# zbqq/neus2

Hardware: AMD Instinct MI355X
Metric: training samples/sec (compacted NeuS2 training samples, DTU-scan24-shaped synthetic, base.json) (higher is better)
Workload: dtype fp16 MFMA (fp32 accumulate) / fp32 optimizer; 1 GPU; NeuS2 train step, Config S, base.json L=14 T=2^19 W=64, Nc=2^18/GPU, R=2^18/GPU fixed, all 14 levels active (network trained 800 steps before the warm-up); global_batch=262144, rays_per_gpu=262144, parallelism=dp1, prepare_steps=800, levels_active=14

## Files before the change

### include/neus2_hip.h

```cpp
#ifndef NEUS2_HIP_H
#define NEUS2_HIP_H

#include <stdint.h>

#ifdef __cplusplus
extern "C" {
#endif

typedef struct NeusTestbed NeusTestbed;

typedef struct NeusNetworkConfig {
	uint32_t n_levels;
	uint32_t n_features_per_level;
	uint32_t log2_hashmap_size;
	uint32_t base_resolution;
	float per_level_scale;
	float top_resolution;
	float valid_level_scale;
	float base_valid_level_scale;
	uint32_t base_training_step;
	uint32_t n_neurons;
	uint32_t n_density_hidden;
	uint32_t n_rgb_hidden;
	float learning_rate, beta1, beta2, epsilon, l2_reg;
// ... 147 lines not shown
	float learning_rate_factor;
} NeusOptimizerState;
int neus_testbed_get_optimizer_state(NeusTestbed* tb, NeusOptimizerState* st, float* m1, float* m2, uint32_t* steps, uint16_t* ema_half);
int neus_testbed_set_optimizer_state(NeusTestbed* tb, const NeusOptimizerState* st, const float* m1, const float* m2, const uint32_t* steps,
                                     const uint16_t* ema_half);
int neus_testbed_set_training_options(NeusTestbed* tb, const NeusTrainingOptions* opts);
int neus_testbed_set_progressive_inference(NeusTestbed* tb, int mode, const uint32_t* chunk_ends, uint32_t n_ends);
int neus_testbed_ray_counts(NeusTestbed* tb, uint32_t n, uint32_t* nreq, uint32_t* ccount, uint32_t* numsteps );
int neus_debug_time_kernel(NeusTestbed* tb, int kernel, int variant, int iters, float* ms_out);
int neus_testbed_time_kernel(NeusTestbed* tb, int kernel, int iters, float* ms_out, uint32_t* units_out);
int neus_debug_march_stats(NeusTestbed* tb, uint32_t n, uint32_t* out);
int neus_debug_march_profile(NeusTestbed* tb, unsigned long long* out, uint32_t max_waves, uint32_t* n_waves);
int neus_debug_scatter_stats(NeusTestbed* tb, uint64_t* records_per_level, uint32_t* max_region);
int neus_debug_scatter_parts(NeusTestbed* tb, uint32_t* parts_per_level );
int neus_debug_grid_scatter(NeusTestbed* tb, void* hip_stream, uint32_t n_cap, const uint32_t* n_valid, const float* coords,
                            uint32_t coord_stride, uint32_t valid_level, const void* dLdenc, const void* genc, const float* v,
                            float* grid_grad_out);
int neus_debug_exclusive_scan(void* hip_stream, const uint32_t* in, uint32_t* out, uint32_t n, int reps, uint32_t* failures);
int neus_debug_scan_giveup(void* hip_stream, const uint32_t* in, uint32_t* out, uint32_t n, uint32_t* failures);
int neus_debug_inject_health(NeusTestbed* tb, uint32_t flags);
int neus_debug_set_lds_fill(NeusTestbed* tb, uint32_t pattern);
int neus_debug_set_lds_fill_all(NeusTestbed* tb, uint32_t pattern);
int neus_debug_set_xcd_shift(NeusTestbed* tb, uint32_t n_blocks);
int neus_debug_get_batch(NeusTestbed* tb, float* coords_out, uint16_t* dl_dout_out, float* loss_out);
int neus_debug_denorm_probe(int device, uint32_t n, uint32_t launches, uint64_t* stats);
int neus_debug_get_buffer(NeusTestbed* tb, int id, uint64_t offset, uint64_t nbytes, void* host);
int neus_debug_replay_loss_grad(NeusTestbed* tb, uint16_t* dl_dout_out);
int neus_debug_sample_rays_round0(NeusTestbed* tb, void* stream, uint32_t n_rays, uint32_t n_rays_total, uint64_t rng_state, uint64_t rng_inc,
                                  uint32_t max_samples, const uint8_t* bitfield, float* rays, uint32_t* numsteps, float* coords,
                                  uint32_t* counters_out, uint32_t chunk_end, uint32_t* list, uint32_t* list_len, uint32_t lds_fill);
int neus_testbed_stream(NeusTestbed* tb, void** hip_stream);
int neus_testbed_synchronize(NeusTestbed* tb);
#define NEUS_N_PHASES 10
int neus_testbed_set_profiling(NeusTestbed* tb, int on);
int neus_testbed_kernel_times(NeusTestbed* tb, float* ms_out );
int neus_testbed_set_infer_timing(NeusTestbed* tb, int on);
int neus_testbed_infer_timing(NeusTestbed* tb, double* ms_total, uint64_t* launches, uint64_t* steps);
int neus_testbed_set_exchange_timing(NeusTestbed* tb, int on);
int neus_testbed_exchange_timing(NeusTestbed* tb, double* exposed_ms_total, double* span_ms_total, uint64_t* steps);

int neus_nccl_unique_id(uint8_t* out );
int neus_testbed_init_data_parallel(NeusTestbed* tb, int rank, int world, const uint8_t* unique_id );
#define NEUS_DP_FORCE_COLLECTIVES 1
int neus_testbed_init_data_parallel_ex(NeusTestbed* tb, int rank, int world, const uint8_t* unique_id, uint32_t flags);
typedef struct NeusDataParallelInfo {
	uint32_t rank, world;
// ... 81 lines not shown
```

### neus2_amd/_lib.py

```python
from __future__ import annotations

import ctypes as C
import os

_HERE = os.path.dirname(os.path.abspath(__file__))
LIB_PATH = os.environ.get("NEUS2_HIP_LIB") or os.path.join(_HERE, "libneus2_hip.so")


class NeusNetworkConfig(C.Structure):
    _fields_ = [
        ("n_levels", C.c_uint32), ("n_features_per_level", C.c_uint32), ("log2_hashmap_size", C.c_uint32),
        ("base_resolution", C.c_uint32), ("per_level_scale", C.c_float), ("top_resolution", C.c_float),
        ("valid_level_scale", C.c_float), ("base_valid_level_scale", C.c_float), ("base_training_step", C.c_uint32),
        ("n_neurons", C.c_uint32), ("n_density_hidden", C.c_uint32), ("n_rgb_hidden", C.c_uint32),
        ("learning_rate", C.c_float), ("beta1", C.c_float), ("beta2", C.c_float), ("epsilon", C.c_float), ("l2_reg", C.c_float),
        ("ema_decay", C.c_float), ("decay_start", C.c_uint32), ("decay_interval", C.c_uint32), ("decay_base", C.c_float),
        ("ek_loss_weight", C.c_float), ("mask_loss_weight", C.c_float), ("anneal_end", C.c_uint32), ("batch_size", C.c_uint32),
        ("sdf_bias", C.c_float), ("density_grid_decay", C.c_float), ("seed", C.c_uint32), ("fixed_rays_per_batch", C.c_uint32),
        ("predict_global_movement", C.c_uint32), ("global_movement_steps", C.c_uint32), ("finetune_global_movement", C.c_uint32),
        ("reset_density_grid_after_global_movement", C.c_uint32), ("after_learning_rate", C.c_float),
        ("gm_learning_rate", C.c_float), ("gm_beta1", C.c_float), ("gm_beta2", C.c_float), ("gm_epsilon", C.c_float),
        ("gm_decay_start", C.c_uint32), ("gm_decay_interval", C.c_uint32), ("gm_decay_base", C.c_float),
    ]

# ... 60 lines not shown
        ("depth_supervision_lambda", C.c_float),
    ]


class NeusOptimizerState(C.Structure):
    _fields_ = [("n_params", C.c_uint32), ("current_step", C.c_uint32), ("learning_rate", C.c_float),
                ("learning_rate_factor", C.c_float)]


class NeusModuleInfo(C.Structure):
    _fields_ = [("n_params", C.c_uint64), ("n_input_dims", C.c_uint32), ("n_output_dims", C.c_uint32),
                ("param_precision", C.c_int32), ("output_precision", C.c_int32), ("gradient_precision", C.c_int32),
                ("batch_capacity", C.c_uint32), ("n_levels", C.c_uint32), ("grid_offset", C.c_uint64),
                ("per_level_scale", C.c_float)]


EXPORTS = [
    "neus_last_error", "neus_abi_version", "neus_device_count", "neus_device_synchronize",
    "neus_testbed_create", "neus_testbed_destroy", "neus_testbed_set_dataset", "neus_testbed_reload_network",
    "neus_testbed_layout", "neus_testbed_train", "neus_testbed_get_stats", "neus_testbed_get_params",
    "neus_testbed_set_params", "neus_testbed_get_gradients", "neus_testbed_get_ema_params",
    "neus_testbed_get_half_params",
    "neus_testbed_get_density_grid", "neus_testbed_set_density_grid", "neus_testbed_restore_state", "neus_testbed_get_rng", "neus_testbed_render", "neus_testbed_sdf_on_grid",
    "neus_testbed_marching_cubes", "neus_testbed_mc_density", "neus_testbed_get_mesh", "neus_testbed_mesh_vertex_colors", "neus_mc_table", "neus_prepare_image_rgba8", "neus_testbed_ray_counts", "neus_debug_time_kernel", "neus_debug_march_stats", "neus_debug_exclusive_scan", "neus_debug_scan_giveup", "neus_debug_inject_health", "neus_debug_set_lds_fill", "neus_debug_set_lds_fill_all", "neus_debug_set_xcd_shift", "neus_debug_denorm_probe", "neus_debug_get_batch", "neus_debug_get_buffer", "neus_debug_replay_loss_grad", "neus_debug_sample_rays_round0", "neus_debug_march_profile", "neus_debug_scatter_stats", "neus_debug_scatter_parts", "neus_debug_grid_scatter", "neus_testbed_time_kernel", "neus_testbed_stream",
    "neus_testbed_synchronize", "neus_testbed_set_profiling", "neus_testbed_kernel_times", "neus_testbed_set_infer_timing", "neus_testbed_infer_timing",
    "neus_testbed_set_exchange_timing", "neus_testbed_exchange_timing",
    "neus_nccl_unique_id", "neus_testbed_init_data_parallel", "neus_testbed_init_data_parallel_ex",
    "neus_testbed_data_parallel_info", "neus_testbed_set_exchange_overlap", "neus_local_group_create", "neus_local_group_destroy",
    "neus_testbed_init_local_group", "neus_host_group_create", "neus_host_group_destroy", "neus_testbed_init_host_group", "neus_debug_host_group_allreduce",
    "neus_grid_encode", "neus_net_forward", "neus_net_backward", "neus_sample_rays", "neus_loss_compact",
    "neus_optimizer_step", "neus_fill_rollover", "neus_occ_update", "neus_mfma_probe",
    "neus_testbed_next_frame", "neus_testbed_get_movement", "neus_testbed_set_movement", "neus_testbed_frame_state",
    "neus_testbed_change_frame", "neus_testbed_prepare_for_test", "neus_testbed_get_training_options",
    "neus_testbed_set_training_options", "neus_testbed_saved_transform", "neus_testbed_get_optimizer_state",
    "neus_testbed_set_optimizer_state", "neus_testbed_set_progressive_inference",
    "neus_module_create_network", "neus_module_create_nerf_network", "neus_module_create_encoding", "neus_module_create_network_with_input_encoding", "neus_module_destroy", "neus_context_destroy",
    "neus_module_info", "neus_module_hyperparams", "neus_module_set_training_step", "neus_module_set_indeed_batch_size",
    "neus_module_initialize_params", "neus_module_inference", "neus_module_forward", "neus_module_backward",
    "neus_module_backward_backward_input",
    "neus_net_backward_pos", "neus_delta_apply", "neus_delta_backward",
]

ABI_VERSION = 7

_lib = None


# ... 29 lines not shown
```

### neus2_amd/csrc/grid.hip

```cpp
#include "kernels.h"
#include "grid_common.h"
#include <algorithm>
#include <vector>

namespace neus {

__device__ __forceinline__ uint32_t load_n(const uint32_t* n_ptr, uint32_t n_fixed) { return n_ptr ? *n_ptr : n_fixed; }

__global__ void __launch_bounds__(256) k_grid_encode(
	const uint32_t* __restrict__ n_ptr, uint32_t n_fixed, uint32_t ld,
	const float* __restrict__ coords, uint32_t coord_stride,
	const GridLevels gl, uint32_t valid_level,
	const half_t* __restrict__ grid, uint32_t* __restrict__ enc, float* __restrict__ dydx, EncodeRollover ro) {
	const uint32_t n = load_n(n_ptr, n_fixed);
	const uint32_t l = blockIdx.y;
	const half_t* gp = grid + (size_t)gl.offset[l] * 2;
	const uint32_t n_in = ro.n_in_ptr ? min(*ro.n_in_ptr, ro.n_elements) : 0xffffffffu;
	for (uint32_t i = blockIdx.x * blockDim.x + threadIdx.x; i < n; i += gridDim.x * blockDim.x) {
		const uint32_t src = i < n_in ? i : i % n_in;
		if (l == 0 && i != src) {
			for (uint32_t k = 0; k < coord_stride; ++k) ro.coords[(size_t)i * coord_stride + k] = coords[(size_t)src * coord_stride + k];
#pragma unroll
			for (int k = 0; k < OUT_W; ++k) {
				const float r = (float)ro.dL_dout[(size_t)src * OUT_W + k];
				ro.dL_dout[(size_t)i * OUT_W + k] = (half_t)(r * n_in / ro.n_elements);
			}
		}
		if (l > valid_level) {
			enc[(size_t)l * ld + i] = 0u;
			if (dydx) {
#pragma unroll
				for (int k = 0; k < 6; ++k) dydx[(size_t)(6 * l + k) * ld + i] = 0.0f;
			}
			continue;
		}
		const float* c = coords + (size_t)src * coord_stride;
		LevelSetup s = level_setup(gl, l, c[0], c[1], c[2]);
		h2 v[8];
		gather_corners(s, gp, v);
		const h2 out = interp_features(s, v);
// ... 76 lines not shown
__device__ __forceinline__ unsigned long long rec_fix(float v, uint32_t k) {
	const float s = __uint_as_float((127u + (uint32_t)SB_FIX_BITS - k) << 23);
	return (unsigned long long)__float2ll_rn(fminf(fmaxf(v, -65504.0f), 65504.0f) * s);
}
__device__ __forceinline__ float fix_to_float(unsigned long long v) { return (float)((double)(long long)v * (1.0 / 274877906944.0)); }

struct ScatterLevel { LevelSetup s; float dl0, dl1, g0, g1, vin[3]; uint32_t off; };
__device__ __forceinline__ void corner_contribution(const ScatterLevel& L, uint32_t idx, uint32_t& gidx, float& a0, float& a1) {
	float wc = 1.f;
#pragma unroll
	for (int d = 0; d < 3; ++d) wc *= (idx & (1u << d)) ? L.s.pos[d] : 1.f - L.s.pos[d];
	float w2 = 0.f;
#pragma unroll
	for (int gd = 0; gd < 3; ++gd) {
		float t = L.vin[gd];
#pragma unroll
		for (int d = 0; d < 3; ++d) if (d != gd) t *= (idx & (1u << d)) ? L.s.pos[d] : 1.f - L.s.pos[d];
		w2 += (idx & (1u << gd)) ? t : -t;
	}
	a0 = L.dl0 * wc + L.g0 * w2;
	a1 = L.dl1 * wc + L.g1 * w2;
	const uint32_t gx = L.s.g[0] + (idx & 1), gy = L.s.g[1] + ((idx >> 1) & 1), gz = L.s.g[2] + ((idx >> 2) & 1);
	gidx = L.off + grid_index(L.s.hsize, L.s.res, gx, gy, gz);
}
__device__ __forceinline__ ScatterLevel scatter_level_ab(const GridLevels& gl, uint32_t l, float x, float y, float z, uint32_t a, uint32_t b2,
                                                         const float4 vv) {
	ScatterLevel L;
	L.s = level_setup(gl, l, x, y, z);
	const h2 d1 = *(const h2*)&a, g2 = *(const h2*)&b2;
	L.dl0 = (float)d1[0]; L.dl1 = (float)d1[1]; L.g0 = (float)g2[0]; L.g1 = (float)g2[1];
	L.vin[0] = L.s.scale * vv.x; L.vin[1] = L.s.scale * vv.y; L.vin[2] = L.s.scale * vv.z;
	L.off = gl.offset[l];
	return L;
}
__device__ __forceinline__ ScatterLevel scatter_level(const GridLevels& gl, uint32_t l, float x, float y, float z, uint32_t ic, uint32_t ld,
                                                      const uint32_t* __restrict__ dLdenc, const uint32_t* __restrict__ g, const float4 vv) {
	ScatterLevel L;
	L.s = level_setup(gl, l, x, y, z);
	const uint32_t a = dLdenc[(size_t)l * ld + ic], b2 = g[(size_t)l * ld + ic];
	const h2 d1 = *(const h2*)&a, g2 = *(const h2*)&b2;
	L.dl0 = (float)d1[0]; L.dl1 = (float)d1[1]; L.g0 = (float)g2[0]; L.g1 = (float)g2[1];
	L.vin[0] = L.s.scale * vv.x; L.vin[1] = L.s.scale * vv.y; L.vin[2] = L.s.scale * vv.z;
	L.off = gl.offset[l];
	return L;
}

// ... 207 lines not shown
			const uint32_t ek = re[idx];
			if (ek != ~0u) {
				const uint32_t e = ek & 0xffffffu;
				const uint32_t lb = (e >> SB_SHIFT) - b_first;
				const uint32_t pos = base[lb] + rs[idx];
				st_i[pos] = (uint16_t)((e & (SB_SIZE - 1)) | (ek >> 24) << SB_SHIFT);
				st_g[pos] = rg[idx];
				st_b[pos] = (uint16_t)lb;
			}
		}
		__syncthreads();
		const uint32_t total = base[nlb];
		for (uint32_t r = threadIdx.x; r < total; r += blockDim.x) {
			const uint32_t lb = st_b[r];
			const uint32_t gp = cursor[lb] + (r - base[lb]);
			w.rec_i[gp] = st_i[r];
			w.rec_g[gp] = __builtin_bit_cast(h2, st_g[r]);
		}
		if (threadIdx.x == 0) { carry_b = b_first + nlb - 1; carry_v = cursor[nlb - 1] + cnt[nlb - 1]; }
	}
}

constexpr uint32_t RT_STRIDE = SB_LEVEL_BUCKETS + 1;
template <int BS>
__global__ void __launch_bounds__(BS) k_scatter_bin_r(const uint32_t* __restrict__ n_ptr, uint32_t n_fixed, uint32_t ld,
                                                        const float* __restrict__ coords, uint32_t coord_stride, const GridLevels gl,
                                                        uint32_t valid_level, const uint32_t* __restrict__ dLdenc, const uint32_t* __restrict__ g,
                                                        const float4* __restrict__ v4, ScatterWork w) {
	__shared__ uint32_t cnt[SB_LEVEL_BUCKETS], base[SB_LEVEL_BUCKETS + 1];
	__shared__ uint16_t st_i[BS * 8];
	__shared__ uint32_t st_g[BS * 8];
	const uint32_t blk = blockIdx.x, lane = threadIdx.x & 63;
	const uint32_t n = load_n(n_ptr, n_fixed);
	const uint32_t i = blk * blockDim.x + threadIdx.x;
	const bool ok = i < n;
	const uint32_t ic = ok ? i : 0;
	const float* c = coords + (size_t)ic * coord_stride;
	const float x = c[0], y = c[1], z = c[2];
	const float4 vv = v4[ic];
	const uint32_t n_lv = min(gl.n_levels, valid_level + 1);
	const uint32_t lstep = gridDim.y;
	uint32_t a_cur = dLdenc[(size_t)blockIdx.y * ld + ic], g_cur = g[(size_t)blockIdx.y * ld + ic];
	for (uint32_t l = blockIdx.y; l < n_lv; l += lstep) {
		const uint32_t ln = min(l + lstep, n_lv - 1);
		const uint32_t a_next = dLdenc[(size_t)ln * ld + ic], g_next = g[(size_t)ln * ld + ic];
		const uint32_t off = gl.offset[l], size = gl.offset[l + 1] - off;
		const uint32_t nlb = (size + SB_SIZE - 1) >> SB_SHIFT;
		const bool few = size <= 4 * SB_SIZE;
		for (uint32_t k = threadIdx.x; k < nlb; k += blockDim.x) cnt[k] = 0;
		__syncthreads();
		const ScatterLevel L = scatter_level_ab(gl, l, x, y, z, a_cur, g_cur, vv);
		a_cur = a_next; g_cur = g_next;
		uint32_t re[8], rs[8], rg[8];
#pragma unroll
		for (uint32_t idx = 0; idx < 8; ++idx) {
			uint32_t gidx; float a0, a1;
			corner_contribution(L, idx, gidx, a0, a1);
			const bool emit = wave_run_sum(gidx, a0, a1, ok);
			const uint32_t e = gidx - off, lb = e >> SB_SHIFT;
			uint32_t sl = 0;
			if (few) sl = wave_bucket_slot(cnt, lb, emit);
			else if (emit) sl = atomicAdd(&cnt[lb], 1u);
			const uint32_t kx = rec_scale_exp(a0, a1);
			re[idx] = emit ? e | kx << 24 : ~0u;
			rs[idx] = sl;
			rg[idx] = rec_value(a0, a1, kx);
		}
		__syncthreads();
		if (threadIdx.x < 64) {
			uint32_t total = 0;
			for (uint32_t k0 = 0; k0 < nlb; k0 += 64) {
				const uint32_t k = k0 + lane;
				const uint32_t v = k < nlb ? cnt[k] : 0u;
				const uint32_t incl = wave_incl_sum(v);
				if (k < nlb) base[k] = total + incl - v;
				total += wave_lane_value(incl, 63);
			}
			if (lane == 0) base[nlb] = total;
		}
		__syncthreads();
#pragma unroll
		for (uint32_t idx = 0; idx < 8; ++idx) {
// ... 287 lines not shown
	if (m) k_enc_rows<<<(uint32_t)((m + 255) / 256), 256, 0, s>>>(n, L, ld, nullptr, nullptr, 1u, paired, rows);
}
void launch_grad_to_half(hipStream_t s, uint32_t n, const float* g, half_t* out, bool accumulate) {
	if (n) k_grad_to_half<<<(n + 255) / 256, 256, 0, s>>>(n, g, out, accumulate ? 1u : 0u);
}
void launch_enc_input_grad(hipStream_t s, uint32_t n, uint32_t ld, uint32_t L, const half_t* dLdy, const float* dydx, float* dLdx, uint32_t stride) {
	if (n) k_enc_input_grad<<<(n + 255) / 256, 256, 0, s>>>(n, ld, L, (const uint32_t*)dLdy, dydx, dLdx, stride);
}
void launch_enc_ddLdoutput(hipStream_t s, uint32_t n, uint32_t ld, uint32_t L, const float* ddx, const float* dydx, half_t* out, float4* v4) {
	if (n) k_enc_ddLdoutput<<<(n + 255) / 256, 256, 0, s>>>(n, ld, L, ddx, dydx, (uint32_t*)out, v4);
}
uint32_t grid_ddx_active_levels(const GridLevels& gl, uint32_t valid_level) { return valid_level >= gl.n_levels ? gl.n_levels : valid_level + 1; }
void launch_grid_ddx_sum(hipStream_t s, uint32_t n, uint32_t n_active, const float* partial, float* dLdx) {
	if (n) k_grid_ddx_sum<<<(n + 255) / 256, 256, 0, s>>>(n, n_active, partial, dLdx);
}
void launch_grid_ddx(hipStream_t s, uint32_t n, uint32_t ld, const float* coords, const GridLevels& gl, uint32_t valid_level, const half_t* grid,
                     const half_t* g, const float* ddx, float* partial, float* dLdx) {
	if (!n) return;
	const uint32_t na = grid_ddx_active_levels(gl, valid_level);
	const uint32_t gx = std::min<uint32_t>((n + 255) / 256, 4096);
	if (na) k_grid_ddx<<<dim3(gx, na), 256, 0, s>>>(n, ld, coords, gl, grid, (const uint32_t*)g, ddx, partial);
	launch_grid_ddx_sum(s, n, na, partial, dLdx);
}
void launch_grid_encode(hipStream_t s, const uint32_t* n_ptr, uint32_t n_fixed, uint32_t ld, const float* coords, uint32_t coord_stride,
                        const GridLevels& gl, uint32_t valid_level, const half_t* grid, uint32_t* enc, float* dydx, uint32_t grid_x,
                        const EncodeRollover* ro) {
	if (!grid_x) return;
	const EncodeRollover r = ro ? *ro : EncodeRollover{nullptr, 0u, nullptr, nullptr};
	dbg_lds_gate(s);
	k_grid_encode<<<dim3(grid_x, gl.n_levels), 256, 0, s>>>(n_ptr, n_fixed, ld, coords, coord_stride, gl, valid_level, grid, enc, dydx, r);
}
size_t scatter_records_capacity(uint32_t n_cap, uint32_t n_levels) { return (size_t)n_cap * n_levels * 8; }
std::vector<uint32_t> scatter_accum_jobs(const GridLevels& gl, uint32_t n_buckets, uint32_t& n_split) {
	std::vector<uint32_t> jobs;
	n_split = 0;
	for (uint32_t b = 0; b < n_buckets; ++b) {
		uint32_t smin = 0xffffffffu;
		for (uint32_t l = 0; l < gl.n_levels; ++l)
			if (gl.offset[l] < (b + 1) * SB_SIZE && gl.offset[l + 1] > b * SB_SIZE) smin = std::min(smin, gl.offset[l + 1] - gl.offset[l]);
		const uint32_t parts = smin == 0xffffffffu ? 1u : std::max(1u, std::min(32u, (uint32_t)((32ull * SB_SIZE) / std::max(1u, smin))));
		const uint32_t slot = parts > 1 ? n_split++ : 0u;
		for (uint32_t p = 0; p < parts; ++p) { jobs.push_back(b); jobs.push_back(p); jobs.push_back(parts); jobs.push_back(slot); }
	}
	return jobs;
}
std::vector<uint32_t> scatter_region_jobs(const GridLevels& gl, uint32_t& n_split, std::vector<uint32_t>& jobs_before_level) {
	std::vector<uint32_t> jobs;
	n_split = 0;
	jobs_before_level.assign(gl.n_levels + 1, 0u);
	for (uint32_t l = 0; l < gl.n_levels; ++l) {
		const uint32_t size = gl.offset[l + 1] - gl.offset[l], nlb = (size + SB_SIZE - 1) / SB_SIZE;
		if (nlb > SB_LEVEL_BUCKETS) throw std::runtime_error("hash-grid level table too large for the scatter's per-level buckets");
		const uint32_t parts = std::max(1u, std::min(32u, (uint32_t)((32ull * SB_SIZE) / std::max(1u, size))));
		for (uint32_t k = 0; k < nlb; ++k) {
			const uint32_t slot = parts > 1 ? n_split++ : 0u;
			for (uint32_t p = 0; p < parts; ++p) { jobs.push_back(l); jobs.push_back(k); jobs.push_back(p | (parts << 16)); jobs.push_back(slot); }
		}
		jobs_before_level[l + 1] = (uint32_t)(jobs.size() / 4);
	}
	return jobs;
}
uint32_t scatter_n_buckets(const GridLevels& gl) {
	for (uint32_t l = 0; l < gl.n_levels; ++l)
		if (((gl.offset[l + 1] - 1) >> SB_SHIFT) - (gl.offset[l] >> SB_SHIFT) + 1 > SB_LEVEL_BUCKETS)
			throw std::runtime_error("hash-grid level table too large for the scatter's per-level buckets");
	return (gl.offset[gl.n_levels] + SB_SIZE - 1) >> SB_SHIFT;
}
static inline uint32_t accum_blocks(uint32_t n, uint32_t xg) { return (n + 8 * xg - 1) / (8 * xg) * (8 * xg); }
void launch_grid_scatter(hipStream_t s, const uint32_t* n_ptr, uint32_t n_fixed, uint32_t ld, const float* coords, uint32_t coord_stride,
                         const GridLevels& gl, uint32_t valid_level, const half_t* dLdenc, const half_t* g, const float4* v, float* grads,
                         const ScatterWork& w, void* scan_tmp, size_t scan_tmp_bytes, const ScatterSplit* split) {
	if (w.mode == 2) {
		const uint32_t n_lv = std::min(gl.n_levels, valid_level + 1);
		const dim3 grid(w.n_chunks, w.level_groups ? std::min(w.level_groups, n_lv) : n_lv);
		dbg_lds_gate(s);
		if (w.chunk == 1024)
			k_scatter_bin_r<1024><<<grid, 1024, 0, s>>>(n_ptr, n_fixed, ld, coords, coord_stride, gl, valid_level, (const uint32_t*)dLdenc,
			                                            (const uint32_t*)g, v, w);
		else if (w.chunk == 256)
			k_scatter_bin_r<256><<<grid, 256, 0, s>>>(n_ptr, n_fixed, ld, coords, coord_stride, gl, valid_level, (const uint32_t*)dLdenc,
			                                          (const uint32_t*)g, v, w);
		else
			k_scatter_bin_r<512><<<grid, 512, 0, s>>>(n_ptr, n_fixed, ld, coords, coord_stride, gl, valid_level, (const uint32_t*)dLdenc,
			                                          (const uint32_t*)g, v, w);
		const uint32_t n_act = std::min(valid_level + 1, gl.n_levels);
		if (!split) {
			const uint32_t nj = std::min(w.n_jobs2, w.jobs2_before[n_act]);
			dbg_lds_gate(s);
			if (nj) k_scatter_accum_r<<<accum_blocks(nj, w.xcd_group), 64 * SC_WAVES, 0, s>>>(w, gl, grads, w.chunk * 8, 0u, nj, w.xcd_group);
			return;
		}
		uint32_t lo = 0;
		for (uint32_t gi = 0; gi < split->n_groups && lo < n_act; ++gi) {
			const uint32_t hi = gi + 1 == split->n_groups ? n_act : std::min(split->level_end[gi], n_act);
			if (hi <= lo) continue;
			const uint32_t j0 = std::min(w.n_jobs2, w.jobs2_before[lo]), j1 = std::min(w.n_jobs2, w.jobs2_before[hi]);
			dbg_lds_gate(s);
			if (j1 > j0)
				k_scatter_accum_r<<<accum_blocks(j1 - j0, w.xcd_group), 64 * SC_WAVES, 0, s>>>(w, gl, grads, w.chunk * 8, j0, j1 - j0, w.xcd_group);
			if (split->done) split->done(lo, hi);
			lo = hi;
		}
		return;
	}
	if (w.mode == 0) {
		const size_t nb = (size_t)w.n_active * w.n_chunks;
		if (w.chunk == 1024)
// ... 27 lines not shown
```

### neus2_amd/csrc/grid_common.h

```cpp
#pragma once
#include "common.h"

namespace neus {

struct LevelSetup { float pos[3]; uint32_t g[3]; float scale; uint32_t hsize, res; };

__device__ __forceinline__ LevelSetup level_setup(float scale, uint32_t res, uint32_t hsize, float x, float y, float z) {
	LevelSetup s;
	s.scale = scale; s.res = res; s.hsize = hsize;
	const float in[3] = {x, y, z};
#pragma unroll
	for (int d = 0; d < 3; ++d) {
		float p = __builtin_fmaf(in[d], s.scale, 0.5f);
		float fl = floorf(p);
		s.g[d] = (uint32_t)(int)fl;
		s.pos[d] = p - fl;
	}
	return s;
}
__device__ __forceinline__ LevelSetup level_setup(const GridLevels& gl, uint32_t l, float x, float y, float z) {
	return level_setup(gl.scale[l], gl.res[l], gl.offset[l + 1] - gl.offset[l], x, y, z);
}

__device__ __forceinline__ void gather_corners(const LevelSetup& s, const half_t* __restrict__ gp, h2 v[8]) {
#pragma unroll
	for (uint32_t idx = 0; idx < 8; ++idx) {
		const uint32_t gx = s.g[0] + (idx & 1), gy = s.g[1] + ((idx >> 1) & 1), gz = s.g[2] + ((idx >> 2) & 1);
		const uint32_t e = grid_index(s.hsize, s.res, gx, gy, gz);
		v[idx] = *(const h2*)(gp + 2 * (size_t)e);
	}
}

__device__ __forceinline__ h2 interp_features(const LevelSetup& s, const h2 v[8]) {
	half_t r0 = (half_t)0.f, r1 = (half_t)0.f;
#pragma unroll
	for (uint32_t idx = 0; idx < 8; ++idx) {
		float w = 1.f;
#pragma unroll
		for (int d = 0; d < 3; ++d) w *= (idx & (1u << d)) ? s.pos[d] : 1.f - s.pos[d];
		r0 = (half_t)((float)r0 + (float)(half_t)(w * (float)v[idx][0]));
		r1 = (half_t)((float)r1 + (float)(half_t)(w * (float)v[idx][1]));
	}
	h2 out; out[0] = r0; out[1] = r1;
	return out;
}

__device__ __forceinline__ void interp_dydx(const LevelSetup& s, const h2 v[8], float gr[2][3]) {
#pragma unroll
	for (int f = 0; f < 2; ++f)
#pragma unroll
		for (int d = 0; d < 3; ++d) gr[f][d] = 0.f;
#pragma unroll
// ... 39 lines not shown
```

### neus2_amd/csrc/kernels.h

```cpp
#pragma once
#include <functional>
#include <vector>
#include "common.h"

namespace neus {

struct MlpPtrs {
	const half_t* d0;  const half_t* d1;
	const half_t* r0;  const half_t* r1;  const half_t* r2;
	const half_t* d0T; const half_t* d1T;
	const half_t* r0T; const half_t* r1T; const half_t* r2T;
	const half_t* d0p; const half_t* d0Tp;
	const half_t* var;
	float sdf_bias;
};

struct TrainBufs {
	half_t* d1_delta;
	half_t* dLdenc; half_t* genc;
	float4* v;
	float* var_grad;
	float* var_partial;
	float indeed_batch;
	float4* dpos;
// ... 108 lines not shown
	float ema_decay, ema_debias_old, ema_debias_new;
	uint32_t optimize_matrix, optimize_non_matrix;
	const float* bias_tab;
	uint32_t bias_converged;
	float inv_loss_scale;
	uint32_t pow2_scale;
	uint32_t skip_ema_h;
	const uint32_t* abort;
};
void launch_adam_bias_table(hipStream_t s, float beta1, float beta2, float* tab);

struct StepCounterArgs { StepState* st; uint32_t target_batch, max_samples, world, fixed_rays; const uint32_t* eval_cnt; uint32_t n_eval; };
struct AdamTranspose {
	uint32_t n;
	uint32_t off[5], rows[5], cols[5];
	half_t* dst[5];
	int32_t inv[48];
	half_t* d0p; half_t* d0Tp; uint32_t din, W;
};
struct TransposeJob { const half_t* src; half_t* dst; uint32_t rows, cols; };
struct TransposeJobs { TransposeJob j[8]; uint32_t n; };

struct EncodeRollover { const uint32_t* n_in_ptr; uint32_t n_elements; half_t* dL_dout; float* coords; };
void launch_grid_encode(hipStream_t s, const uint32_t* n_ptr, uint32_t n_fixed, uint32_t ld, const float* coords, uint32_t coord_stride,
                        const GridLevels& gl, uint32_t valid_level, const half_t* grid, uint32_t* enc, float* dydx, uint32_t grid_x, const EncodeRollover* ro = nullptr);
size_t scatter_records_capacity(uint32_t n_cap, uint32_t n_levels);
uint32_t scatter_n_buckets(const GridLevels& gl);
struct ScatterSplit { uint32_t n_groups; uint32_t level_end[8]; std::function<void(uint32_t, uint32_t)> done; };
void launch_grid_scatter(hipStream_t s, const uint32_t* n_ptr, uint32_t n_cap, uint32_t ld, const float* coords, uint32_t coord_stride,
                         const GridLevels& gl, uint32_t valid_level, const half_t* dLdenc, const half_t* g, const float4* v, float* grads,
                         const ScatterWork& w, void* scan_tmp, size_t scan_tmp_bytes, const ScatterSplit* split = nullptr);
bool mlp_supported(uint32_t n_levels, uint32_t width);
void mlp_din_permutation(uint32_t L, int32_t* perm );
struct InferAlpha {
	float4* sa; float* ekt; float cos_anneal; uint32_t dt_const; uint32_t* n_long;
	uint32_t xcd_parts = 0;
};
void launch_nerf_infer(hipStream_t s, uint32_t L, uint32_t W, const uint32_t* n_ptr, uint32_t n_fixed, const float* coords, const GridLevels& gl,
                       uint32_t valid_level, const half_t* grid, const MlpPtrs& w, half_t* out, uint32_t blocks,
                       const uint32_t* idx = nullptr , const InferAlpha* ia = nullptr);
void launch_nerf_density(hipStream_t s, uint32_t L, uint32_t W, uint32_t n, const float* pos, const GridLevels& gl, uint32_t valid_level,
                         const half_t* grid, const MlpPtrs& w, float* density);
struct OccSampling {
	uint32_t n_u, n_nu, lo;
	uint64_t rng_u_state, rng_u_inc, rng_nu_state, rng_nu_inc;
	uint32_t step, n_cascades;
// ... 224 lines not shown
```

### neus2_amd/csrc/testbed.cpp

```cpp
#include <rocprofiler-sdk-roctx/roctx.h>
#include "kernels.h"
#include "scan_lookback.h"
#include "json_lite.h"
#include "hostgroup.h"
#include "options.h"
#include "../../include/neus2_hip.h"

#include <rccl/rccl.h>

#include <algorithm>
#include <atomic>
#include <cstdio>
#include <functional>
#include <chrono>
#include <cmath>
#include <condition_variable>
#include <mutex>
#include <cstdlib>
#include <cstring>
#include <memory>
#include <random>
#include <stdexcept>
#include <string>
#include <vector>
// ... 2617 lines not shown
	});
}
int neus_debug_sample_rays_round0(NeusTestbed* tb, void* stream, uint32_t n_rays, uint32_t n_rays_total, uint64_t rng_state, uint64_t rng_inc,
                                  uint32_t max_samples, const uint8_t* bitfield, float* rays, uint32_t* numsteps, float* coords, uint32_t* counters_out,
                                  uint32_t chunk_end, uint32_t* list, uint32_t* list_len, uint32_t lds_fill) {
	return guard([&] {
		if (chunk_end == 0 || !list || !list_len) throw std::runtime_error("sample_rays_round0: chunk_end > 0, list and list_len required");
		sample_rays_impl(tb, stream, n_rays, 0u, 1u, n_rays_total, rng_state, rng_inc, max_samples, bitfield, rays, numsteps, coords, counters_out,
		                 chunk_end, list, list_len, lds_fill);
	});
}
int neus_debug_scan_giveup(void* stream, const uint32_t* in, uint32_t* out, uint32_t n, uint32_t* failures) {
	return guard([&] {
		hipStream_t s = (hipStream_t)stream;
		ScanTemp tmp; tmp.alloc(scan_temp_bytes(n) + 256); scan_temp_reset(s, tmp.p);
		debug_scan_skip_first_tile(s, tmp.p, in, out, n);
		HIP_CHECK(hipStreamSynchronize(s));
		*failures = scan_failures(tmp.p);
	});
}
int neus_debug_set_lds_fill(NeusTestbed* tb, uint32_t pattern) { return guard([&] { tb->dbg_lds_fill = pattern; }); }
int neus_debug_set_lds_fill_all(NeusTestbed* tb, uint32_t pattern) { return guard([&] { tb->dbg_lds_fill_all = pattern; }); }
int neus_debug_set_xcd_shift(NeusTestbed* tb, uint32_t n_blocks) { return guard([&] { tb->dbg_xcd_shift = n_blocks; }); }
int neus_debug_denorm_probe(int device, uint32_t n, uint32_t launches, uint64_t* stats) {
	return guard([&] {
		if (!stats || n == 0) throw std::runtime_error("neus_debug_denorm_probe: bad argument");
		HIP_CHECK(hipSetDevice(device));
		hipStream_t s = nullptr;
		HIP_CHECK(hipStreamCreateWithFlags(&s, hipStreamNonBlocking));
		try { debug_denorm_probe(s, n, launches, stats); } catch (...) { (void)hipStreamDestroy(s); throw; }
		HIP_CHECK(hipStreamDestroy(s));
	});
}
int neus_debug_get_buffer(NeusTestbed* tb, int id, uint64_t offset, uint64_t nbytes, void* host) {
	return guard([&] {
		if (!tb->have_net) throw std::runtime_error("no network");
		const void* p = nullptr;
		size_t cap = 0;
		auto pick = [&](const void* q, size_t bytes) { p = q; cap = bytes; };
		switch (id) {
		case 0: pick(tb->l_sa.p, tb->l_sa.n * 16); break;
		case 1: pick(tb->l_ekt.p, tb->l_ekt.n * 4); break;
		case 2: pick(tb->l_ck4.p, tb->l_ck4.n * 16); break;
		case 3: pick(tb->l_cke.p, tb->l_cke.n * 4); break;
		case 4: pick(tb->l_racc.p, tb->l_racc.n * 16); break;
		case 5: pick(tb->l_rgr.p, tb->l_rgr.n * 16); break;
// ... 1322 lines not shown
```

Baseline: 334.1 million samples/s.

## Add direct-index fast paths for grid encode and scatter binning kernels

Adds DIRECT template variants of the grid encode and scatter-bin kernels, used when every level's dense or hashed index can be computed with cheap masks or min-subtract instead of a generic modulo. The index is computed once per corner set and byte-offset addressing is used. In scatter binning, a per-wave run plan checks whether all eight corners share the same run boundaries and, if so, does one shared DPP segmented-sum schedule instead of eight separate wave_run_sum calls. Coordinate loads are also moved inside the level loop to lower register pressure. This adds code complexity, host-side eligibility checks and a debug switch back to the generic path.

```diff
diff --git a/include/neus2_hip.h b/include/neus2_hip.h
--- a/include/neus2_hip.h
+++ b/include/neus2_hip.h
@@ -193,6 +193,7 @@
 int neus_debug_set_lds_fill(NeusTestbed* tb, uint32_t pattern);
 int neus_debug_set_lds_fill_all(NeusTestbed* tb, uint32_t pattern);
 int neus_debug_set_xcd_shift(NeusTestbed* tb, uint32_t n_blocks);
+int neus_debug_set_grid_generic(uint32_t on);
 int neus_debug_get_batch(NeusTestbed* tb, float* coords_out, uint16_t* dl_dout_out, float* loss_out);
 int neus_debug_denorm_probe(int device, uint32_t n, uint32_t launches, uint64_t* stats);
 int neus_debug_get_buffer(NeusTestbed* tb, int id, uint64_t offset, uint64_t nbytes, void* host);
diff --git a/neus2_amd/_lib.py b/neus2_amd/_lib.py
--- a/neus2_amd/_lib.py
+++ b/neus2_amd/_lib.py
@@ -106,7 +106,7 @@
     "neus_testbed_set_params", "neus_testbed_get_gradients", "neus_testbed_get_ema_params",
     "neus_testbed_get_half_params",
     "neus_testbed_get_density_grid", "neus_testbed_set_density_grid", "neus_testbed_restore_state", "neus_testbed_get_rng", "neus_testbed_render", "neus_testbed_sdf_on_grid",
-    "neus_testbed_marching_cubes", "neus_testbed_mc_density", "neus_testbed_get_mesh", "neus_testbed_mesh_vertex_colors", "neus_mc_table", "neus_prepare_image_rgba8", "neus_testbed_ray_counts", "neus_debug_time_kernel", "neus_debug_march_stats", "neus_debug_exclusive_scan", "neus_debug_scan_giveup", "neus_debug_inject_health", "neus_debug_set_lds_fill", "neus_debug_set_lds_fill_all", "neus_debug_set_xcd_shift", "neus_debug_denorm_probe", "neus_debug_get_batch", "neus_debug_get_buffer", "neus_debug_replay_loss_grad", "neus_debug_sample_rays_round0", "neus_debug_march_profile", "neus_debug_scatter_stats", "neus_debug_scatter_parts", "neus_debug_grid_scatter", "neus_testbed_time_kernel", "neus_testbed_stream",
+    "neus_testbed_marching_cubes", "neus_testbed_mc_density", "neus_testbed_get_mesh", "neus_testbed_mesh_vertex_colors", "neus_mc_table", "neus_prepare_image_rgba8", "neus_testbed_ray_counts", "neus_debug_time_kernel", "neus_debug_march_stats", "neus_debug_exclusive_scan", "neus_debug_scan_giveup", "neus_debug_inject_health", "neus_debug_set_lds_fill", "neus_debug_set_lds_fill_all", "neus_debug_set_xcd_shift", "neus_debug_set_grid_generic", "neus_debug_denorm_probe", "neus_debug_get_batch", "neus_debug_get_buffer", "neus_debug_replay_loss_grad", "neus_debug_sample_rays_round0", "neus_debug_march_profile", "neus_debug_scatter_stats", "neus_debug_scatter_parts", "neus_debug_grid_scatter", "neus_testbed_time_kernel", "neus_testbed_stream",
     "neus_testbed_synchronize", "neus_testbed_set_profiling", "neus_testbed_kernel_times", "neus_testbed_set_infer_timing", "neus_testbed_infer_timing",
     "neus_testbed_set_exchange_timing", "neus_testbed_exchange_timing",
     "neus_nccl_unique_id", "neus_testbed_init_data_parallel", "neus_testbed_init_data_parallel_ex",
diff --git a/neus2_amd/csrc/grid.hip b/neus2_amd/csrc/grid.hip
--- a/neus2_amd/csrc/grid.hip
+++ b/neus2_amd/csrc/grid.hip
@@ -7,6 +7,7 @@
 
 __device__ __forceinline__ uint32_t load_n(const uint32_t* n_ptr, uint32_t n_fixed) { return n_ptr ? *n_ptr : n_fixed; }
 
+template <bool DIRECT>
 __global__ void __launch_bounds__(256) k_grid_encode(
 	const uint32_t* __restrict__ n_ptr, uint32_t n_fixed, uint32_t ld,
 	const float* __restrict__ coords, uint32_t coord_stride,
@@ -16,6 +17,55 @@
 	const uint32_t l = blockIdx.y;
 	const half_t* gp = grid + (size_t)gl.offset[l] * 2;
 	const uint32_t n_in = ro.n_in_ptr ? min(*ro.n_in_ptr, ro.n_elements) : 0xffffffffu;
+	if constexpr (DIRECT) {
+		const uint32_t i0 = blockIdx.x * blockDim.x + threadIdx.x, istep = gridDim.x * blockDim.x;
+		char* encl = (char*)(enc + (size_t)l * ld);
+		char* dyl = dydx ? (char*)(dydx + (size_t)6 * l * ld) : nullptr;
+		if (l > valid_level) {
+			for (uint32_t i = i0; i < n; i += istep) {
+				*(uint32_t*)(encl + (i << 2)) = 0u;
+				if (dydx) {
+#pragma unroll
+					for (uint32_t k = 0; k < 6; ++k) *(float*)(dyl + ((k * ld + i) << 2)) = 0.0f;
+				}
+			}
+		} else {
+			const char* tab = (const char*)gp;
+			const float scale = gl.scale[l];
+			const uint32_t res = gl.res[l], hsize = gl.offset[l + 1] - gl.offset[l];
+			const bool dense = (gl.dense_bits >> l) & 1u;
+			for (uint32_t i = i0; i < n; i += istep) {
+				const uint32_t src = i < n_in ? i : i % n_in;
+				const float* c = (const float*)((const char*)coords + ((src * coord_stride) << 2));
+				const LevelSetup s = level_setup(scale, res, hsize, c[0], c[1], c[2]);
+				uint32_t e[8];
+				corner_entries(s, dense, e);
+				h2 v[8];
+#pragma unroll
+				for (int k = 0; k < 8; ++k) v[k] = *(const h2*)(tab + (e[k] << 2));
+				const h2 out = interp_features(s, v);
+				*(uint32_t*)(encl + (i << 2)) = *(const uint32_t*)&out;
+				if (dydx) {
+					float gr[2][3];
+					interp_dydx(s, v, gr);
+#pragma unroll
+					for (uint32_t k = 0; k < 6; ++k) *(float*)(dyl + ((k * ld + i) << 2)) = gr[k / 3][k % 3];
+				}
+			}
+		}
+		if (l == 0 && n_in < n) {
+			for (uint32_t i = n_in + i0; i < n; i += istep) {
+				const uint32_t src = i % n_in;
+				for (uint32_t k = 0; k < coord_stride; ++k) ro.coords[(size_t)i * coord_stride + k] = coords[(size_t)src * coord_stride + k];
+#pragma unroll
+				for (int k = 0; k < OUT_W; ++k) {
+					const float r = (float)ro.dL_dout[(size_t)src * OUT_W + k];
+					ro.dL_dout[(size_t)i * OUT_W + k] = (half_t)(r * n_in / ro.n_elements);
+				}
+			}
+		}
+		return;
+	}
 	for (uint32_t i = blockIdx.x * blockDim.x + threadIdx.x; i < n; i += gridDim.x * blockDim.x) {
 		const uint32_t src = i < n_in ? i : i % n_in;
 		if (l == 0 && i != src) {
@@ -138,6 +188,19 @@
 	a1 = L.dl1 * wc + L.g1 * w2;
 	const uint32_t gx = L.s.g[0] + (idx & 1), gy = L.s.g[1] + ((idx >> 1) & 1), gz = L.s.g[2] + ((idx >> 2) & 1);
 	gidx = L.off + grid_index(L.s.hsize, L.s.res, gx, gy, gz);
+}
+__device__ __forceinline__ void corner_values(const ScatterLevel& L, uint32_t idx, float& a0, float& a1) {
+#pragma clang fp contract(off)
+	float f[3];
+#pragma unroll
+	for (int d = 0; d < 3; ++d) f[d] = (idx & (1u << d)) ? L.s.pos[d] : 1.f - L.s.pos[d];
+	const float wc = f[0] * f[1] * f[2];
+	const float u0 = L.vin[0] * f[1], u1 = L.vin[1] * f[0], u2 = L.vin[2] * f[0];
+	float w2 = (idx & 1u) ? 0.f + u0 * f[2] : __builtin_fmaf(-f[2], u0, 0.f);
+	w2 = (idx & 2u) ? w2 + u1 * f[2] : __builtin_fmaf(-f[2], u1, w2);
+	w2 = (idx & 4u) ? w2 + u2 * f[1] : __builtin_fmaf(-f[1], u2, w2);
+	a0 = __builtin_fmaf(L.dl0, wc, L.g0 * w2);
+	a1 = __builtin_fmaf(L.dl1, wc, L.g1 * w2);
 }
 __device__ __forceinline__ ScatterLevel scatter_level_ab(const GridLevels& gl, uint32_t l, float x, float y, float z, uint32_t a, uint32_t b2,
                                                          const float4 vv) {
@@ -391,7 +454,67 @@
 }
 
 constexpr uint32_t RT_STRIDE = SB_LEVEL_BUCKETS + 1;
-template <int BS>
+
+struct RunPlan { bool same, none, tail, c[6]; };
+__device__ __forceinline__ RunPlan level_run_plan(const ScatterLevel& L, bool dense, bool ok, uint32_t e[8]) {
+	const uint32_t lane = threadIdx.x & 63;
+	corner_entries(L.s, dense, e);
+	uint64_t heads[8];
+#pragma unroll
+	for (uint32_t idx = 0; idx < 8; ++idx) {
+		if (!ok) e[idx] = 0xffffffffu;
+		heads[idx] = __ballot(dpp_u32<DPP_WAVE_SHR1>(~e[idx], e[idx]) != e[idx]);
+	}
+	RunPlan P;
+	P.same = true;
+#pragma unroll
+	for (uint32_t idx = 1; idx < 8; ++idx) P.same = P.same && heads[idx] == heads[0];
+	const uint64_t hd = heads[0];
+	P.none = hd == ~0ull;
+	const uint32_t rs = 63u - (uint32_t)__clzll(hd & ((2ull << lane) - 1ull));
+	const uint32_t r0 = lane & ~15u;
+	P.c[0] = lane - r0 >= 1u && lane - 1u >= rs;
+	P.c[1] = lane - r0 >= 2u && lane - 2u >= rs;
+	P.c[2] = lane - r0 >= 4u && lane - 4u >= rs;
+	P.c[3] = lane - r0 >= 8u && lane - 8u >= rs;
+	P.c[4] = (r0 == 16u || r0 == 48u) && rs < r0;
+	P.c[5] = lane >= 32u && rs < 32u;
+	P.tail = lane == 63u || ((hd >> (lane + 1u)) & 1ull);
+	return P;
+}
+__device__ __forceinline__ uint32_t corner_run_sums(const RunPlan& P, const ScatterLevel& L, bool ok, const uint32_t e[8], float a0[8], float a1[8]) {
+#pragma unroll
+	for (uint32_t k = 0; k < 8; ++k) {
+		corner_values(L, k, a0[k], a1[k]);
+		if (!ok) a0[k] = a1[k] = 0.f;
+	}
+	if (!P.same) {
+		uint32_t em = 0;
+#pragma unroll
+		for (uint32_t k = 0; k < 8; ++k) em |= wave_run_sum(e[k], a0[k], a1[k], ok) ? 1u << k : 0u;
+		return em;
+	}
+	const uint32_t all = 0xffu;
+	if (P.none) return ok ? all : 0u;
+#define NEUS_SEG_STEPG(CTRL, MASK, C)                                                                    \
+	if (__ballot(C)) {                                                                                   \
+		_Pragma("unroll") for (uint32_t k = 0; k < 8; ++k) {                                             \
+			const float t0 = dpp_f32<CTRL, MASK>(0.f, a0[k]), t1 = dpp_f32<CTRL, MASK>(0.f, a1[k]);      \
+			a0[k] = (C) ? a0[k] + t0 : a0[k];                                                            \
+			a1[k] = (C) ? a1[k] + t1 : a1[k];                                                            \
+		}                                                                                                \
+	}
+	NEUS_SEG_STEPG(DPP_ROW_SHR + 1, 0xf, P.c[0])
+	NEUS_SEG_STEPG(DPP_ROW_SHR + 2, 0xf, P.c[1])
+	NEUS_SEG_STEPG(DPP_ROW_SHR + 4, 0xf, P.c[2])
+	NEUS_SEG_STEPG(DPP_ROW_SHR + 8, 0xf, P.c[3])
+	NEUS_SEG_STEPG(DPP_BCAST15, 0xa, P.c[4])
+	NEUS_SEG_STEPG(DPP_BCAST31, 0xc, P.c[5])
+#undef NEUS_SEG_STEPG
+	return ok && P.tail ? all : 0u;
+}
+
+template <int BS, bool DIRECT>
 __global__ void __launch_bounds__(BS) k_scatter_bin_r(const uint32_t* __restrict__ n_ptr, uint32_t n_fixed, uint32_t ld,
                                                         const float* __restrict__ coords, uint32_t coord_stride, const GridLevels gl,
                                                         uint32_t valid_level, const uint32_t* __restrict__ dLdenc, const uint32_t* __restrict__ g,
@@ -404,9 +527,13 @@
 	const uint32_t i = blk * blockDim.x + threadIdx.x;
 	const bool ok = i < n;
 	const uint32_t ic = ok ? i : 0;
-	const float* c = coords + (size_t)ic * coord_stride;
-	const float x = c[0], y = c[1], z = c[2];
-	const float4 vv = v4[ic];
+	float x = 0.f, y = 0.f, z = 0.f;
+	float4 vv = make_float4(0.f, 0.f, 0.f, 0.f);
+	if constexpr (!DIRECT) {
+		const float* c = coords + (size_t)ic * coord_stride;
+		x = c[0]; y = c[1]; z = c[2];
+		vv = v4[ic];
+	}
 	const uint32_t n_lv = min(gl.n_levels, valid_level + 1);
 	const uint32_t lstep = gridDim.y;
 	uint32_t a_cur = dLdenc[(size_t)blockIdx.y * ld + ic], g_cur = g[(size_t)blockIdx.y * ld + ic];
@@ -418,15 +545,36 @@
 		const bool few = size <= 4 * SB_SIZE;
 		for (uint32_t k = threadIdx.x; k < nlb; k += blockDim.x) cnt[k] = 0;
 		__syncthreads();
+		if constexpr (DIRECT) {
+			uint32_t icl = ic;
+			asm volatile("" : "+v"(icl));
+			const float* c = coords + (size_t)icl * coord_stride;
+			x = c[0]; y = c[1]; z = c[2];
+			vv = v4[icl];
+		}
 		const ScatterLevel L = scatter_level_ab(gl, l, x, y, z, a_cur, g_cur, vv);
 		a_cur = a_next; g_cur = g_next;
 		uint32_t re[8], rs[8], rg[8];
+		uint32_t ce[8], em = 0;
+		float ca0[8], ca1[8];
+		if constexpr (DIRECT) {
+			const RunPlan rp = level_run_plan(L, (gl.dense_bits >> l) & 1u, ok, ce);
+			em = corner_run_sums(rp, L, ok, ce, ca0, ca1);
+		}
 #pragma unroll
 		for (uint32_t idx = 0; idx < 8; ++idx) {
-			uint32_t gidx; float a0, a1;
-			corner_contribution(L, idx, gidx, a0, a1);
-			const bool emit = wave_run_sum(gidx, a0, a1, ok);
-			const uint32_t e = gidx - off, lb = e >> SB_SHIFT;
+			uint32_t e; float a0, a1;
+			bool emit;
+			if constexpr (DIRECT) {
+				e = ce[idx]; a0 = ca0[idx]; a1 = ca1[idx];
+				emit = (em >> idx) & 1u;
+			} else {
+				uint32_t gidx;
+				corner_contribution(L, idx, gidx, a0, a1);
+				emit = wave_run_sum(gidx, a0, a1, ok);
+				e = gidx - off;
+			}
+			const uint32_t lb = e >> SB_SHIFT;
 			uint32_t sl = 0;
 			if (few) sl = wave_bucket_slot(cnt, lb, emit);
 			else if (emit) sl = atomicAdd(&cnt[lb], 1u);
@@ -760,13 +908,41 @@
 	if (na) k_grid_ddx<<<dim3(gx, na), 256, 0, s>>>(n, ld, coords, gl, grid, (const uint32_t*)g, ddx, partial);
 	launch_grid_ddx_sum(s, n, na, partial, dLdx);
 }
+uint32_t g_dbg_grid_generic = 0;
+static bool grid_levels_direct_index(const GridLevels& gl) {
+	if (g_dbg_grid_generic) return false;
+	for (uint32_t l = 0; l < gl.n_levels; ++l) {
+		const uint64_t r = gl.res[l], hs = gl.offset[l + 1] - gl.offset[l];
+		if (hs == 0) return false;
+		if ((gl.dense_bits >> l) & 1u) {
+			if (r * r * r > hs || r + r * r + r * r * r >= 2 * hs) return false;
+		} else {
+			uint32_t stride = gl.res[l];
+			if (stride <= hs) stride *= gl.res[l];
+			if (stride <= hs) stride *= gl.res[l];
+			if (!(hs < stride) || (hs & (hs - 1)) != 0) return false;
+		}
+	}
+	return true;
+}
+static bool encode_direct_ok(const GridLevels& gl, uint32_t ld, uint32_t coord_stride) {
+	if (!grid_levels_direct_index(gl)) return false;
+	const uint64_t lim = 1ull << 31;
+	if (6ull * gl.n_levels * ld >= lim || 24ull * ld >= lim || 4ull * ld * coord_stride >= lim) return false;
+	for (uint32_t l = 0; l < gl.n_levels; ++l)
+		if (4ull * (gl.offset[l + 1] - gl.offset[l]) >= lim) return false;
+	return true;
+}
 void launch_grid_encode(hipStream_t s, const uint32_t* n_ptr, uint32_t n_fixed, uint32_t ld, const float* coords, uint32_t coord_stride,
                         const GridLevels& gl, uint32_t valid_level, const half_t* grid, uint32_t* enc, float* dydx, uint32_t grid_x,
                         const EncodeRollover* ro) {
 	if (!grid_x) return;
 	const EncodeRollover r = ro ? *ro : EncodeRollover{nullptr, 0u, nullptr, nullptr};
 	dbg_lds_gate(s);
-	k_grid_encode<<<dim3(grid_x, gl.n_levels), 256, 0, s>>>(n_ptr, n_fixed, ld, coords, coord_stride, gl, valid_level, grid, enc, dydx, r);
+	if (encode_direct_ok(gl, ld, coord_stride))
+		k_grid_encode<true><<<dim3(grid_x, gl.n_levels), 256, 0, s>>>(n_ptr, n_fixed, ld, coords, coord_stride, gl, valid_level, grid, enc, dydx, r);
+	else
+		k_grid_encode<false><<<dim3(grid_x, gl.n_levels), 256, 0, s>>>(n_ptr, n_fixed, ld, coords, coord_stride, gl, valid_level, grid, enc, dydx, r);
 }
 size_t scatter_records_capacity(uint32_t n_cap, uint32_t n_levels) { return (size_t)n_cap * n_levels * 8; }
 std::vector<uint32_t> scatter_accum_jobs(const GridLevels& gl, uint32_t n_buckets, uint32_t& n_split) {
@@ -812,15 +988,18 @@
 		const uint32_t n_lv = std::min(gl.n_levels, valid_level + 1);
 		const dim3 grid(w.n_chunks, w.level_groups ? std::min(w.level_groups, n_lv) : n_lv);
 		dbg_lds_gate(s);
-		if (w.chunk == 1024)
-			k_scatter_bin_r<1024><<<grid, 1024, 0, s>>>(n_ptr, n_fixed, ld, coords, coord_stride, gl, valid_level, (const uint32_t*)dLdenc,
-			                                            (const uint32_t*)g, v, w);
-		else if (w.chunk == 256)
-			k_scatter_bin_r<256><<<grid, 256, 0, s>>>(n_ptr, n_fixed, ld, coords, coord_stride, gl, valid_level, (const uint32_t*)dLdenc,
-			                                          (const uint32_t*)g, v, w);
-		else
-			k_scatter_bin_r<512><<<grid, 512, 0, s>>>(n_ptr, n_fixed, ld, coords, coord_stride, gl, valid_level, (const uint32_t*)dLdenc,
-			                                          (const uint32_t*)g, v, w);
+#define NEUS_BIN_R(BS, DIRECT) \
+	k_scatter_bin_r<BS, DIRECT><<<grid, BS, 0, s>>>(n_ptr, n_fixed, ld, coords, coord_stride, gl, valid_level, (const uint32_t*)dLdenc, (const uint32_t*)g, v, w)
+		if (grid_levels_direct_index(gl)) {
+			if (w.chunk == 1024) NEUS_BIN_R(1024, true);
+			else if (w.chunk == 256) NEUS_BIN_R(256, true);
+			else NEUS_BIN_R(512, true);
+		} else {
+			if (w.chunk == 1024) NEUS_BIN_R(1024, false);
+			else if (w.chunk == 256) NEUS_BIN_R(256, false);
+			else NEUS_BIN_R(512, false);
+		}
+#undef NEUS_BIN_R
 		const uint32_t n_act = std::min(valid_level + 1, gl.n_levels);
 		if (!split) {
 			const uint32_t nj = std::min(w.n_jobs2, w.jobs2_before[n_act]);
diff --git a/neus2_amd/csrc/grid_common.h b/neus2_amd/csrc/grid_common.h
--- a/neus2_amd/csrc/grid_common.h
+++ b/neus2_amd/csrc/grid_common.h
@@ -28,6 +28,30 @@
 		const uint32_t gx = s.g[0] + (idx & 1), gy = s.g[1] + ((idx >> 1) & 1), gz = s.g[2] + ((idx >> 2) & 1);
 		const uint32_t e = grid_index(s.hsize, s.res, gx, gy, gz);
 		v[idx] = *(const h2*)(gp + 2 * (size_t)e);
+	}
+}
+
+__device__ __forceinline__ void corner_entries(const LevelSetup& s, bool dense, uint32_t e[8]) {
+	const uint32_t hs = s.hsize;
+	if (dense) {
+		const uint32_t rr = s.res * s.res;
+		const uint32_t y0 = s.g[1] * s.res, y1 = y0 + s.res, z0 = s.g[2] * rr, z1 = z0 + rr;
+		const uint32_t yz[4] = {y0 + z0, y1 + z0, y0 + z1, y1 + z1};
+		if (__builtin_expect(s.g[0] >= s.res || s.g[1] >= s.res || s.g[2] >= s.res, 0)) {
+#pragma unroll
+			for (uint32_t idx = 0; idx < 8; ++idx) e[idx] = (s.g[0] + (idx & 1) + yz[idx >> 1]) % hs;
+		} else {
+#pragma unroll
+			for (uint32_t idx = 0; idx < 8; ++idx) {
+				const uint32_t ed = s.g[0] + (idx & 1) + yz[idx >> 1];
+				e[idx] = min(ed, ed - hs);
+			}
+		}
+	} else {
+		const uint32_t y0 = s.g[1] * 2654435761u, y1 = y0 + 2654435761u, z0 = s.g[2] * 805459861u, z1 = z0 + 805459861u;
+		const uint32_t yz[4] = {y0 ^ z0, y1 ^ z0, y0 ^ z1, y1 ^ z1};
+#pragma unroll
+		for (uint32_t idx = 0; idx < 8; ++idx) e[idx] = ((s.g[0] + (idx & 1)) ^ yz[idx >> 1]) & (hs - 1u);
 	}
 }
 
diff --git a/neus2_amd/csrc/kernels.h b/neus2_amd/csrc/kernels.h
--- a/neus2_amd/csrc/kernels.h
+++ b/neus2_amd/csrc/kernels.h
@@ -154,6 +154,7 @@
 struct TransposeJobs { TransposeJob j[8]; uint32_t n; };
 
 struct EncodeRollover { const uint32_t* n_in_ptr; uint32_t n_elements; half_t* dL_dout; float* coords; };
+extern uint32_t g_dbg_grid_generic;
 void launch_grid_encode(hipStream_t s, const uint32_t* n_ptr, uint32_t n_fixed, uint32_t ld, const float* coords, uint32_t coord_stride,
                         const GridLevels& gl, uint32_t valid_level, const half_t* grid, uint32_t* enc, float* dydx, uint32_t grid_x, const EncodeRollover* ro = nullptr);
 size_t scatter_records_capacity(uint32_t n_cap, uint32_t n_levels);
diff --git a/neus2_amd/csrc/testbed.cpp b/neus2_amd/csrc/testbed.cpp
--- a/neus2_amd/csrc/testbed.cpp
+++ b/neus2_amd/csrc/testbed.cpp
@@ -2663,6 +2663,7 @@
 int neus_debug_set_lds_fill(NeusTestbed* tb, uint32_t pattern) { return guard([&] { tb->dbg_lds_fill = pattern; }); }
 int neus_debug_set_lds_fill_all(NeusTestbed* tb, uint32_t pattern) { return guard([&] { tb->dbg_lds_fill_all = pattern; }); }
 int neus_debug_set_xcd_shift(NeusTestbed* tb, uint32_t n_blocks) { return guard([&] { tb->dbg_xcd_shift = n_blocks; }); }
+int neus_debug_set_grid_generic(uint32_t on) { return guard([&] { g_dbg_grid_generic = on; }); }
 int neus_debug_denorm_probe(int device, uint32_t n, uint32_t launches, uint64_t* stats) {
 	return guard([&] {
 		if (!stats || n == 0) throw std::runtime_error("neus_debug_denorm_probe: bad argument");
```

Result: faster. 344.1 million samples/s, median of 6 (+3.0%).
